# AKASH2907/pi-consistency-activity-detection

Measured on AMD Instinct MI355X. Metric: train clips/sec (bs=8, 16×224×224, I3D+caps+bv cons) at 1/2/4/8 GPU, higher is better.
Workload: dtype f32 (fp32 operands and fp32 accumulation everywhere; 33 of the 79 conv / input-gradient launches and the 3x3x3 / 1x1x1 weight gradients multiply on the bf16 matrix cores: every fp32 operand as the exact sum of 3 bf16 terms, 6 products on v_mfma_f32_32x32x16_bf16, hi / lo fp32 accumulators -- error v

## Files before the change

### include/picons.h

```cpp
#ifndef PICONS_H
#define PICONS_H
#include <stdint.h>
#ifdef __cplusplus
extern "C" {
#endif

typedef void* pc_stream;

#define PC_OK            0
#define PC_E_ARG        -1
#define PC_E_LAUNCH     -2
#define PC_E_NODEVICE   -3

#define PC_ACT_NONE 0
#define PC_ACT_RELU 1
#define PC_ACT_SIGMOID 2

#define PC_F_ACCUM   1
#define PC_F_BIAS    2
#define PC_F_CSCALE  4
#define PC_F_BNPART  8
#define PC_F_NFAST   16
#define PC_F_TOUT    32
#define PC_F_CI3     64
// ... 91 lines not shown
    pc_wgrad_desc d;
    const float* D; const float* S; float* g;
} pc_wgrad_job;
int pc_conv_wgrad_multi(const pc_wgrad_job* jobs, int njobs, pc_stream s);

int pc_bn_finalize(const float* part, int nparts_per_group, int groups, int C, int64_t count_per_group,
                   const float* gamma, const float* beta, float eps, float momentum,
                   float* running_mean, float* running_var, float* stat, pc_stream s);
int64_t pc_bn_finalize_ws_floats(int nparts_per_group, int groups, int C);
int pc_bn_finalize_ws(const float* part, int nparts_per_group, int groups, int C, int64_t count_per_group,
                      const float* gamma, const float* beta, float eps, float momentum,
                      float* running_mean, float* running_var, float* stat, float* ws, pc_stream s);
int pc_bn_apply(const float* z, int ldz, const float* stat, int C, int64_t rows, int groups, float* y,
                int ldy, int relu, pc_stream s);
int pc_bn_finalize_apply_ok(int nparts_per_group, int C);
int pc_bn_finalize_apply(const float* part, int nparts_per_group, int groups, int C, int64_t count_per_group, const float* gamma, const float* beta,
                         float eps, float momentum, float* running_mean, float* running_var, float* stat, const float* z, int ldz, int64_t rows,
                         float* y, int ldy, int relu, pc_stream s);
int pc_bn_eval_stat(const float* gamma, const float* beta, const float* running_mean,
                    const float* running_var, float eps, int C, float* stat, pc_stream s);
int64_t pc_bn_bwd_ws_floats(int64_t rows, int C, int groups);
int pc_bn_bwd(const float* dy, int lddy, const float* z, int ldz, const float* stat, int C,
              int64_t rows, int groups, int relu, float* dz, int lddz, float* dgamma, float* dbeta,
              int accum, float* ws, pc_stream s);

typedef struct pc_pool_desc {
    int32_t N, Ti, Hi, Wi, C, ldi;
    int32_t To, Ho, Wo, ldo;
    int32_t k[3], s[3], padf[3];
} pc_pool_desc;
int pc_maxpool_fwd(const pc_pool_desc* d, const float* x, float* y, uint8_t* argmax, pc_stream s);
int pc_maxpool_bwd(const pc_pool_desc* d, const float* dy, const uint8_t* argmax, float* dx,
                   int accum, pc_stream s);

int pc_channel_scale(const float* x, int ldx, const float* scale, int N, int64_t pos_per_n, int C,
                     float* y, int ldy, int accum, pc_stream s);
int64_t pc_act_bwd_ws_floats(int64_t rows, int C);
int pc_act_bwd(const float* dy, int lddy, const float* y, int ldy, int act, int C, int64_t rows,
               float* dz, int lddz, float* dbias, int accum, float* ws, pc_stream s);
int pc_ncdhw_to_ndhwc(const void* src, int src_is_f64, int N, int C, int64_t thw, int W, int Cpad,
                      int flipw, float* dst, pc_stream s);
int pc_ndhwc_to_ncdhw(const float* src, int ld, int N, int C, int64_t thw, float* dst, pc_stream s);
int pc_transpose_batched(const float* src, int batch, int R, int Cc, int64_t src_batch_stride,
                         int src_ld, float* dst, int64_t dst_batch_stride, int dst_ld, int accum,
                         pc_stream s);
typedef struct pc_transpose_job {
    uint64_t src, dst;
    int64_t  src_batch_stride, dst_batch_stride;
    int32_t  batch, R, C, src_ld, dst_ld, accum;
    int32_t  nslices, reserved;
    int64_t  slice_stride;
} pc_transpose_job;
int pc_transpose_multi(const pc_transpose_job* jobs, int njobs, pc_stream s);
int pc_col2im(const float* cols, int N, int Ho, int Wo, int KH, int KW, int C, float* dx, int lddx,
              int accum, pc_stream s);
int pc_seg_frame_counts(const float* logits, const float* gt, int64_t nframes, int64_t pix, int32_t* counts, pc_stream s);
int pc_map_accumulate(const int32_t* counts, int64_t nframes, int label, int ncls, int32_t* frame_hits, int32_t* video_hits,
                      int32_t* n_frames, int32_t* n_vids, pc_stream s);
int     pc_val_record_words(int B);
int64_t pc_val_metrics_ws_floats(int B, int64_t pix);
int     pc_val_metrics(const float* output, const float* loc_msk, const float* predicted_action, const int32_t* action, int B, int64_t pix,
                       int C, int32_t* record, float* ws, pc_stream s);
int pc_clip_from_u8(const uint8_t* video, int F, int H, int W, const int32_t* span8, int h0, int w0, int S,
                    const int32_t* rects, int R, float* data, float* aug, float* mask, pc_stream s);
int pc_clip_from_u8_masks(const uint8_t* video, int F, int H, int W, const int32_t* span8, int h0, int w0, int S,
                          const uint8_t* maskframes, const int32_t* valid8, float* data, float* aug, float* mask, float* mask_cls,
// ... 56 lines not shown
    float   bv_wt, gv_wt, wt_loc, wt_cons, wt_ramp;
} pc_loss_desc;
int64_t pc_loss_ws_floats(const pc_loss_desc* d);
int pc_consistency_loss(const pc_loss_desc* d, const float* output, const float* flip_op,
                        const float* seg, const int32_t* labeled, float* scalars, float* d_output,
                        float* d_flip_op, float* mask_bv, float* mask_gv, float* ws, pc_stream s);
int pc_var_mask(const float* pred, const float* flip_pred, int B, int T, int H, int W, int n_frames,
                int use_sig, float* mask, float* ws, pc_stream s);
int pc_grad_mask(const float* pred, int B, int T, int H, int W, float lower, float upper,
                 float* mask, float* ws, pc_stream s);
int pc_spread_loss(const float* x, const float* cls, const int32_t* labeled, int Bn, int C, float m,
                   float wt, float* out, float* dx, pc_stream s);

int pc_adam_step(float* p, const float* g, float* m, float* v, int64_t n, float lr, float b1,
                 float b2, float eps, int step, float gscale, pc_stream s);

typedef struct pc_axis_desc {
    int32_t R, I, O, C;
    int32_t in_split, out_split, act, act_c0, accum;
    int32_t in_sr, in_hi, in_lo, out_sr, out_hi, out_lo;
} pc_axis_desc;
int pc_axis_linear(const pc_axis_desc* d, const float* in, const float* M, const float* bias, float* out, pc_stream s);
int pc_wspec_fwd(const float* in, const float* tw, int A, int B, int KY, int KX, int U, int Ur, float* out, pc_stream s);
int pc_wspec_bwd(const float* dV, const float* tw, int A, int B, int KY, int KX, int U, int Ur, float* kg, pc_stream s);

int pc_wspec_master_fwd(const float* w, const float* tw, int Acnt, int a0, int Atot, int B, int KY, int KX, int U, int Ur,
                        float* out_f, float* out_t, pc_stream s);
int pc_wspec_master_planes(const float* w, const float* tw, int Acnt, int a0, int Atot, int B, int KY, int KX, int U, int Ur,
                           uint16_t* out_f, uint16_t* out_t, int64_t plane_stride, pc_stream s);
int pc_wspec_master_bwd(const float* dV, const float* tw, int Acnt, int a0, int Atot, int B, int KY, int KX, int U, int Ur,
                        float* dw, int accum, pc_stream s);

int pc_tail6_weights(const float* wf, int N, int Ci, float* W5f, float* W5t, pc_stream s);
int pc_tail6_gather(const float* cols, const float* bc, const float* bsm, int N, int It, int Ih, int Iw, float* out, pc_stream s);
int pc_tail6_scatter(const float* dout, int N, int It, int Ih, int Iw, float* dcols, pc_stream s);
int pc_tail6_wgrad_map(const float* dW5, int N, int Ci, float* Gc, pc_stream s);
int pc_tail6_wgrad_map_slices(float* ws, const int32_t* nslices8, int N, int Ci, float* Gc, pc_stream s);
int pc_tail6_bias_sums(const float* dout, int N, int It, int Ih, int Iw, float* sums, pc_stream s);
int64_t pc_tail6_bias_sums_ws_floats(int N, int It, int Ih, int Iw);
int pc_tail6_bias_sums_ws(const float* dout, int N, int It, int Ih, int Iw, float* sums, float* ws, pc_stream s);

typedef struct pc_op {
    int32_t  kind;
    int32_t  i[48];
    float    f[8];
    int32_t  lane;
    uint64_t p[12];
    int64_t  l[4];
} pc_op;
enum {
    PC_OP_CONV = 1, PC_OP_WGRAD, PC_OP_BN_FINALIZE, PC_OP_BN_APPLY, PC_OP_BN_EVAL_STAT, PC_OP_BN_BWD,
    PC_OP_POOL_FWD, PC_OP_POOL_BWD, PC_OP_CHSCALE, PC_OP_ACT_BWD, PC_OP_TO_NDHWC, PC_OP_TO_NCDHW,
    PC_OP_TRANSPOSE, PC_OP_FILL, PC_OP_AXPY, PC_OP_EM_FWD, PC_OP_EM_BWD, PC_OP_CMASK_FWD,
    PC_OP_CMASK_BWD, PC_OP_TAPSUM_FWD, PC_OP_TAPSUM_BWD, PC_OP_LOSS, PC_OP_SPREAD, PC_OP_ADAM,
    PC_OP_TAIL_COMBINE, PC_OP_TAIL_COLSUM, PC_OP_TAIL_GRADS, PC_OP_COL2IM,
    PC_OP_AXIS,
    PC_OP_WSPEC_FWD,
    PC_OP_WSPEC_BWD,
    PC_OP_WSPEC_MASTER_FWD,
    PC_OP_WSPEC_MASTER_BWD,
    PC_OP_TAIL6_WEIGHTS,
    PC_OP_TAIL6_GATHER,
    PC_OP_TAIL6_SCATTER,
    PC_OP_TAIL6_WGRAD_MAP,
    PC_OP_TAIL6_BIAS_SUMS,
    PC_OP_TRANSPOSE_MULTI,
// ... 28 lines not shown
```

### pi-consistency-activity-detection_amd/capi.py

```python
import ctypes as C
import os

import numpy as np

_HERE = os.path.dirname(os.path.abspath(__file__))
DIAG = os.environ.get("PICONS_DIAG_LIB", "0") not in ("", "0")
DIAG_SWITCHES = ("PICONS_CONV_ABLATE", "PICONS_WGRAD_ABLATE", "PICONS_WINO_VARIANT")
LIB_PATH = os.path.join(_HERE, "libpicons_diag.so" if DIAG else "libpicons.so")
if os.environ.get("PICONS_LIB_NAME"):
    LIB_PATH = os.path.join(_HERE, os.path.basename(os.environ["PICONS_LIB_NAME"]))
_lib = None

i32, i64, f32, vp = C.c_int32, C.c_int64, C.c_float, C.c_void_p


class ConvDesc(C.Structure):
    _fields_ = [(n, i32) for n in ("N", "Ti", "Hi", "Wi", "Ci", "ldi", "Tq", "Hq", "Wq", "To", "Ho", "Wo", "Co", "ldo")] + \
               [(n, i32 * 3) for n in ("ostr", "ooff", "istr", "ntap", "ioff0", "istep", "wk0", "wkstep")] + \
               [(n, i32) for n in ("KT", "KH", "KW", "ldw", "act", "flags", "wgstride", "bgstride", "act_c0", "groups")]


class WgradDesc(C.Structure):
    _fields_ = [(n, i32) for n in ("N", "Tq", "Hq", "Wq", "Cd", "ldd", "Ts", "Hs", "Ws", "Cs", "lds")] + \
               [(n, i32 * 3) for n in ("istr", "ntap", "ioff0", "istep", "wk0")] + [(n, i32) for n in ("KT", "KH", "KW", "splitk", "nbatch", "dbstride", "sbstride", "gbstride", "Td", "Hd", "Wd")] + [("doff", i32 * 3), ("flags", i32), ("ws_slices", i32)]
# ... 114 lines not shown
    "pc_clips_from_u8_views": (i32, [vp, i32, i32, i32, i32, C.POINTER(C.c_int32), i32, i32, C.POINTER(C.c_int32), i32, i32, vp, vp]),
    "pc_detect_frames_views_ws_bytes": (i64, [i32, i32, i32]),
    "pc_detect_frames_views": (i32, [vp, i32, i32, i32, i32, C.POINTER(C.c_int32), i32, i32, C.POINTER(C.c_int32), i32, i32, i32, vp, vp, vp, vp]),
    "pc_resize_tables": (i64, [i32, i32, i32, i32, i32, vp, i64]),
    "pc_resize_u8": (i32, [vp, i32, i32, i32, i32, i32, i32, vp, i32, vp, vp]),
    "pc_fill": (i32, [vp, i64, f32, vp]),
    "pc_axpy": (i32, [vp, vp, i64, f32, vp]),
    "pc_em_ws_floats": (i64, [i32, i32, i32]),
    "pc_em_state_floats": (i64, [i32]),
    "pc_em_routing_fwd": (i32, [vp, vp, vp, vp, i32, i32, i32, vp, vp, vp]),
    "pc_em_routing_bwd": (i32, [vp, vp, vp, vp, vp, i32, i32, i32, vp, vp, vp, vp, vp, vp, vp]),
    "pc_class_mask_fwd": (i32, [vp, i32, i32, i32, vp, vp, i32, vp, vp, vp, vp]),
    "pc_class_mask_bwd": (i32, [vp, vp, vp, i32, i32, i32, vp, vp]),
    "pc_tapsum_fwd": (i32, [vp, i32, i32, i32, i32, vp, vp, vp]),
    "pc_tapsum_bwd": (i32, [vp, i32, i32, i32, i32, vp, vp]),
    "pc_loss_ws_floats": (i64, [C.POINTER(LossDesc)]),
    "pc_consistency_loss": (i32, [C.POINTER(LossDesc), vp, vp, vp, vp, vp, vp, vp, vp, vp, vp, vp]),
    "pc_var_mask": (i32, [vp, vp, i32, i32, i32, i32, i32, i32, vp, vp, vp]),
    "pc_grad_mask": (i32, [vp, i32, i32, i32, i32, f32, f32, vp, vp, vp]),
    "pc_spread_loss": (i32, [vp, vp, vp, i32, i32, f32, f32, vp, vp, vp]),
    "pc_adam_step": (i32, [vp, vp, vp, vp, i64, f32, f32, f32, f32, i32, f32, vp]),
    "pc_tail_combine": (i32, [vp, vp, vp, vp, i32, i32, i32, i32, i32, vp, vp, vp, vp]),
    "pc_tail_colsum": (i32, [vp, i32, i64, vp, vp]),
    "pc_tail_grads": (i32, [vp, vp, vp, vp, vp, vp, i32, i32, i32, i32, i32, i32, vp, vp, vp, vp, i32, vp]),
    "pc_tail_grads_ws_floats": (i64, [i32, i32, i32]),
    "pc_tail_grads_ws": (i32, [vp, vp, vp, vp, vp, vp, i32, i32, i32, i32, i32, i32, vp, vp, vp, vp, i32, vp, vp]),
    "pc_axis_linear": (i32, [vp, vp, vp, vp, vp, vp]),
    "pc_wspec_fwd": (i32, [vp, vp, i32, i32, i32, i32, i32, i32, vp, vp]),
    "pc_wspec_bwd": (i32, [vp, vp, i32, i32, i32, i32, i32, i32, vp, vp]),
    "pc_wspec_master_fwd": (i32, [vp, vp, i32, i32, i32, i32, i32, i32, i32, i32, vp, vp, vp]),
    "pc_wspec_master_planes": (i32, [vp, vp, i32, i32, i32, i32, i32, i32, i32, i32, vp, vp, i64, vp]),
    "pc_wspec_master_bwd": (i32, [vp, vp, i32, i32, i32, i32, i32, i32, i32, i32, vp, i32, vp]),
    "pc_tail6_weights": (i32, [vp, i32, i32, vp, vp, vp]),
    "pc_tail6_gather": (i32, [vp, vp, vp, i32, i32, i32, i32, vp, vp]),
    "pc_tail6_scatter": (i32, [vp, i32, i32, i32, i32, vp, vp]),
    "pc_tail6_wgrad_map": (i32, [vp, i32, i32, vp, vp]),
    "pc_tail6_bias_sums": (i32, [vp, i32, i32, i32, i32, vp, vp]),
    "pc_tail6_wgrad_map_slices": (i32, [vp, vp, i32, i32, vp, vp]),
    "pc_tail6_bias_sums_ws_floats": (i64, [i32, i32, i32, i32]),
    "pc_tail6_bias_sums_ws": (i32, [vp, i32, i32, i32, i32, vp, vp, vp]),
    "pc_transpose_multi": (i32, [vp, i32, vp]),
    "pc_run_ops": (i32, [vp, i32, vp]),
    "pc_run_ops_lanes": (i32, [vp, i32, vp, i32]),
    "pc_streams_fanin": (i32, [vp, vp, i32]),
    "pc_release_thread_events": (i32, []),
    "pc_run_ops_timed": (i32, [vp, i32, i32, C.POINTER(f32), C.POINTER(i32), vp, i32]),
    "pc_run_ops_timed_collect": (i32, [C.POINTER(f32), C.POINTER(i32)]),
}
EXPORTS = sorted(_SIGS)


def lib():
    global _lib
    if _lib is None:
        stray = [k for k in DIAG_SWITCHES if os.environ.get(k, "0") not in ("", "0")]
        if stray and not DIAG:
            raise RuntimeError("%s set, but these switches exist only in the diagnostic build of the library (results can be wrong by design): "
                               "`make -C pi-consistency-activity-detection_amd/csrc diag` and PICONS_DIAG_LIB=1, or unset them" % ", ".join(stray))
        if not os.path.exists(LIB_PATH):
            raise RuntimeError("libpicons.so not built (%s): run `python -c 'import __graft_entry__ as g; g.build()'` "
                               "or `make -C pi-consistency-activity-detection_amd/csrc`; there is no CPU fallback" % LIB_PATH)
        L = C.CDLL(LIB_PATH)
        for name, (res, args) in _SIGS.items():
            fn = getattr(L, name)
            fn.restype = res
            fn.argtypes = args
# ... 27 lines not shown
```

### pi-consistency-activity-detection_amd/csrc/api.hip

```cpp
#include "common.h"
#include <string.h>
#include <vector>

static thread_local char g_err[512] = "";

void pc_set_error(const char* fmt, ...) {
    va_list ap;
    va_start(ap, fmt);
    vsnprintf(g_err, sizeof(g_err), fmt, ap);
    va_end(ap);
}

extern "C" const char* pc_last_error(void) { return g_err; }
extern "C" int pc_version(void) { return PC_VERSION; }

extern "C" int pc_transpose_batched(const float*, int, int, int, int64_t, int, float*, int64_t, int, int, pc_stream);

#define P(T, k) ((T)(uintptr_t)op.p[k])

static int run_one(const pc_op& op, pc_stream s) {
    switch (op.kind) {
        case PC_OP_CONV: {
            pc_conv_desc d;
            memcpy(&d, op.i, sizeof(d));
// ... 61 lines not shown
            return pc_transpose_batched(P(const float*, 0), op.i[0], op.i[1], op.i[2], op.l[0], op.i[3], P(float*, 1), op.l[1], op.i[4], op.i[5], s);
        case PC_OP_FILL:
            return pc_fill(P(float*, 0), op.l[0], op.f[0], s);
        case PC_OP_AXPY:
            return pc_axpy(P(float*, 0), P(const float*, 1), op.l[0], op.f[0], s);
        case PC_OP_EM_FWD:
            return pc_em_routing_fwd(P(const float*, 0), P(const float*, 1), P(const float*, 2), P(const float*, 3), op.i[0], op.i[1], op.i[2], P(float*, 4), P(float*, 5), s);
        case PC_OP_EM_BWD:
            return pc_em_routing_bwd(P(const float*, 0), P(const float*, 1), P(const float*, 2), P(const float*, 3), P(const float*, 4), op.i[0], op.i[1],
                                     op.i[2], P(float*, 5), P(float*, 6), P(float*, 7), P(float*, 8), P(float*, 9), P(const float*, 10), s);
        case PC_OP_CMASK_FWD:
            return pc_class_mask_fwd(P(const float*, 0), op.i[0], op.i[1], op.i[2], P(const float*, 1), P(const int32_t*, 2), op.i[3], P(float*, 3),
                                     P(float*, 4), P(float*, 5), s);
        case PC_OP_CMASK_BWD:
            return pc_class_mask_bwd(P(const float*, 0), P(const float*, 1), P(const float*, 2), op.i[0], op.i[1], op.i[2], P(float*, 3), s);
        case PC_OP_TAPSUM_FWD:
            return pc_tapsum_fwd(P(const float*, 0), op.i[0], op.i[1], op.i[2], op.i[3], P(const float*, 1), P(float*, 2), s);
        case PC_OP_TAPSUM_BWD:
            return pc_tapsum_bwd(P(const float*, 0), op.i[0], op.i[1], op.i[2], op.i[3], P(float*, 1), s);
        case PC_OP_LOSS: {
            pc_loss_desc d;
            d.B = op.i[0]; d.T = op.i[1]; d.H = op.i[2]; d.W = op.i[3]; d.bv = op.i[4]; d.gv = op.i[5]; d.n_frames = op.i[6];
            d.predict_maps = op.i[7]; d.jhmdb = op.i[8];
            d.lower_thresh = op.f[0]; d.upper_thresh = op.f[1]; d.bv_wt = op.f[2]; d.gv_wt = op.f[3]; d.wt_loc = op.f[4];
            d.wt_cons = op.f[5]; d.wt_ramp = op.f[6];
            return pc_consistency_loss(&d, P(const float*, 0), P(const float*, 1), P(const float*, 2), P(const int32_t*, 3), P(float*, 4), P(float*, 5),
                                       P(float*, 6), P(float*, 7), P(float*, 8), P(float*, 9), s);
        }
        case PC_OP_SPREAD:
            return pc_spread_loss(P(const float*, 0), P(const float*, 1), P(const int32_t*, 2), op.i[0], op.i[1], op.f[0], op.f[1], P(float*, 3), P(float*, 4), s);
        case PC_OP_ADAM:
            return pc_adam_step(P(float*, 0), P(const float*, 1), P(float*, 2), P(float*, 3), op.l[0], op.f[0], op.f[1], op.f[2], op.f[3], op.i[0], op.f[4], s);
        case PC_OP_TAIL_COMBINE:
            return pc_tail_combine(P(const float*, 0), P(const float*, 1), P(const float*, 2), P(const float*, 3), op.i[0], op.i[1], op.i[2], op.i[3],
                                   op.i[4], P(float*, 4), P(float*, 5), P(float*, 6), s);
        case PC_OP_TAIL_COLSUM:
            return pc_tail_colsum(P(const float*, 0), op.i[0], op.l[0], P(float*, 1), s);
        case PC_OP_TAIL_GRADS:
            return pc_tail_grads_ws(P(const float*, 0), P(const float*, 1), P(const float*, 2), P(const float*, 3), P(const float*, 4), P(const float*, 5),
                                    op.i[0], op.i[1], op.i[2], op.i[3], op.i[4], op.i[5], P(float*, 6), P(float*, 7), P(float*, 8), P(float*, 9), op.i[6],
                                    P(float*, 10), s);
        case PC_OP_COL2IM:
            return pc_col2im(P(const float*, 0), op.i[0], op.i[1], op.i[2], op.i[3], op.i[4], op.i[5], P(float*, 1), op.i[6], op.i[7], s);
        case PC_OP_AXIS: {
            pc_axis_desc d;
            memcpy(&d, op.i, sizeof(d));
            return pc_axis_linear(&d, P(const float*, 0), P(const float*, 1), P(const float*, 2), P(float*, 3), s);
        }
        case PC_OP_WSPEC_FWD:
            return pc_wspec_fwd(P(const float*, 0), P(const float*, 1), op.i[0], op.i[1], op.i[2], op.i[3], op.i[4], op.i[5], P(float*, 2), s);
        case PC_OP_WSPEC_BWD:
            return pc_wspec_bwd(P(const float*, 0), P(const float*, 1), op.i[0], op.i[1], op.i[2], op.i[3], op.i[4], op.i[5], P(float*, 2), s);
        case PC_OP_WSPEC_MASTER_FWD:
            return pc_wspec_master_fwd(P(const float*, 0), P(const float*, 1), op.i[0], op.i[1], op.i[2], op.i[3], op.i[4], op.i[5], op.i[6], op.i[7],
                                       P(float*, 2), P(float*, 3), s);
        case PC_OP_WSPEC_MASTER_BWD:
            return pc_wspec_master_bwd(P(const float*, 0), P(const float*, 1), op.i[0], op.i[1], op.i[2], op.i[3], op.i[4], op.i[5], op.i[6], op.i[7],
                                       P(float*, 2), op.i[8], s);
        case PC_OP_TAIL6_WEIGHTS:
            return pc_tail6_weights(P(const float*, 0), op.i[0], op.i[1], P(float*, 1), P(float*, 2), s);
        case PC_OP_TAIL6_GATHER:
            return pc_tail6_gather(P(const float*, 0), P(const float*, 1), P(const float*, 2), op.i[0], op.i[1], op.i[2], op.i[3], P(float*, 3), s);
        case PC_OP_TAIL6_SCATTER:
            return pc_tail6_scatter(P(const float*, 0), op.i[0], op.i[1], op.i[2], op.i[3], P(float*, 1), s);
        case PC_OP_TAIL6_WGRAD_MAP:
            return op.i[2] ? pc_tail6_wgrad_map_slices(P(float*, 0), &op.i[3], op.i[0], op.i[1], P(float*, 1), s)
// ... 178 lines not shown
```

### pi-consistency-activity-detection_amd/csrc/tail6.hip

```cpp
#include "common.h"
#include <stdlib.h>

namespace {

constexpr int NSLOT = 125, SP = 128, J32 = 32;

__device__ __forceinline__ int npairs(int k5, bool first) { return k5 == 0 || k5 == 4 ? 1 : (k5 == 2 ? (first ? 2 : 3) : 2); }
__device__ __forceinline__ int pair_k4(int k5, bool first, int q) {
    switch (k5) {
        case 0: return 0;
        case 1: return q;
        case 2: return first ? 1 + q : q;
        case 3: return 1 + q;
        default: return 2;
    }
}

__global__ __launch_bounds__(256) void tail6_weights_kernel(const float* __restrict__ wf, int N, int Ci, float* __restrict__ W5f,
                                                            float* __restrict__ W5t) {
    const int64_t total = (int64_t)N * 8 * SP * Ci;
    for (int64_t idx = (int64_t)blockIdx.x * 256 + threadIdx.x; idx < total; idx += (int64_t)gridDim.x * 256) {
        const int ci = (int)(idx % Ci);
        const int slot = (int)((idx / Ci) % SP);
        const int z = (int)((idx / ((int64_t)Ci * SP)) % 8);
        const int n = (int)(idx / ((int64_t)Ci * SP * 8));
        float acc = 0.f;
        if (slot < NSLOT) {
            const int st = slot / 25, sh = (slot / 5) % 5, sw = slot % 5;
            const bool ft = z & 4, fh = z & 2, fw = z & 1;
            const float* base = wf + (size_t)n * J32 * 27 * Ci + ci;
            for (int a = 0; a < npairs(st, ft); ++a)
                for (int b = 0; b < npairs(sh, fh); ++b)
                    for (int c = 0; c < npairs(sw, fw); ++c) {
                        const int ka = pair_k4(st, ft, a), kb = pair_k4(sh, fh, b), kc = pair_k4(sw, fw, c);
                        const int tap = (ka * 3 + kb) * 3 + kc;
                        const int j = ((st - ka) * 3 + (sh - kb)) * 3 + (sw - kc);
                        acc += base[((size_t)j * 27 + tap) * Ci];
                    }
        }
        W5f[idx] = acc;
        W5t[(((size_t)n * 8 + z) * Ci + ci) * SP + slot] = acc;
    }
}

__device__ __forceinline__ int dim_terms(int o, int I, int (&ii)[3], int (&kk)[3]) {
    int n = 0;
#pragma unroll
    for (int k5 = 0; k5 < 5; ++k5) {
        const int t = o + 2 - k5;
        if (t >= 0 && !(t & 1) && (t >> 1) < I) { ii[n] = t >> 1; kk[n] = k5; ++n; }
    }
    return n;
}

__global__ __launch_bounds__(256) void tail6_gather_kernel(const float* __restrict__ cols, const float* __restrict__ bc, const float* __restrict__ bsm,
                                                           int N, int It, int Ih, int Iw, float* __restrict__ out) {
    const int Ot = 2 * It, Oh = 2 * Ih, Ow = 2 * Iw;
    const int64_t total = (int64_t)N * Ot * Oh * Ow;
    const int64_t idx = (int64_t)blockIdx.x * 256 + threadIdx.x;
    if (idx >= total) return;
    const int ow = (int)(idx % Ow), oh = (int)((idx / Ow) % Oh), ot = (int)((idx / ((int64_t)Ow * Oh)) % Ot), n = (int)(idx / ((int64_t)Ow * Oh * Ot));
    int it[3], kt[3], ih[3], kh[3], iw[3], kw[3];
    const int nt = dim_terms(ot, It, it, kt), nh = dim_terms(oh, Ih, ih, kh), nw = dim_terms(ow, Iw, iw, kw);
    float acc = bsm[0];
    for (int a = 0; a < 3; ++a) {
        const int mt = ot + 1 - a;
        if (mt < 0 || mt >= Ot) continue;
        for (int b = 0; b < 3; ++b) {
            const int mh = oh + 1 - b;
            if (mh < 0 || mh >= Oh) continue;
            for (int c = 0; c < 3; ++c) {
                const int mw = ow + 1 - c;
                if (mw < 0 || mw >= Ow) continue;
                acc += bc[n * J32 + (a * 3 + b) * 3 + c];
            }
        }
    }
// ... 171 lines not shown
        else atomicAdd(sums + n * J32 + threadIdx.x, v);
    }
}

__global__ __launch_bounds__(32) void tail6_bias_sums_final_kernel(const float* __restrict__ part, int nb, float* __restrict__ sums) {
    const int n = blockIdx.x, j = threadIdx.x;
    float v = 0.f;
    if (j < 27) {
        const float* q = part + (size_t)n * nb * J32 + j;
        int b = 0;
        for (; b + 14 <= nb; b += 14) {
            float t[14];
#pragma unroll
            for (int u = 0; u < 14; ++u) t[u] = q[(size_t)(b + u) * J32];
#pragma unroll
            for (int u = 0; u < 14; ++u) v += t[u];
        }
        for (; b < nb; ++b) v += q[(size_t)b * J32];
    }
    sums[n * J32 + j] = v;
}

}

extern "C" int pc_tail6_weights(const float* wf, int N, int Ci, float* W5f, float* W5t, pc_stream s) {
    PC_CHECK_ARG(wf && W5f && W5t && N >= 1 && Ci >= 1, "pc_tail6_weights: bad args");
    const int64_t total = (int64_t)N * 8 * SP * Ci;
    int grid = (int)((total + 255) / 256); if (grid > 8192) grid = 8192;
    hipLaunchKernelGGL(tail6_weights_kernel, dim3(grid), dim3(256), 0, (hipStream_t)s, wf, N, Ci, W5f, W5t);
    PC_CHECK_LAUNCH("tail6_weights");
    return PC_OK;
}

extern "C" int pc_tail6_gather(const float* cols, const float* bc, const float* bsm, int N, int It, int Ih, int Iw, float* out, pc_stream s) {
    PC_CHECK_ARG(cols && bc && bsm && out && N >= 1 && It >= 1 && Ih >= 1 && Iw >= 1, "pc_tail6_gather: bad args");
    const int64_t total = (int64_t)N * 8 * It * Ih * Iw;
    PC_CHECK_ARG((total + 255) / 256 < (1ll << 31), "pc_tail6_gather: too large");
    if (((uintptr_t)out & 7) == 0) {
        const dim3 grid((unsigned)((int64_t)N * It * Ih));
        hipLaunchKernelGGL((tail6_gather_rows_kernel<0, 0>), grid, dim3(128), 0, (hipStream_t)s, cols, bc, bsm, N, It, Ih, Iw, out);
        hipLaunchKernelGGL((tail6_gather_rows_kernel<0, 1>), grid, dim3(128), 0, (hipStream_t)s, cols, bc, bsm, N, It, Ih, Iw, out);
        hipLaunchKernelGGL((tail6_gather_rows_kernel<1, 0>), grid, dim3(128), 0, (hipStream_t)s, cols, bc, bsm, N, It, Ih, Iw, out);
        hipLaunchKernelGGL((tail6_gather_rows_kernel<1, 1>), grid, dim3(128), 0, (hipStream_t)s, cols, bc, bsm, N, It, Ih, Iw, out);
    } else {
        hipLaunchKernelGGL(tail6_gather_kernel, dim3((unsigned)cdiv(total, 256)), dim3(256), 0, (hipStream_t)s, cols, bc, bsm, N, It, Ih, Iw, out);
    }
    PC_CHECK_LAUNCH("tail6_gather");
    return PC_OK;
}

extern "C" int pc_tail6_scatter(const float* dout, int N, int It, int Ih, int Iw, float* dcols, pc_stream s) {
    PC_CHECK_ARG(dout && dcols && N >= 1 && It >= 1 && Ih >= 1 && Iw >= 1, "pc_tail6_scatter: bad args");
    const int64_t total = (int64_t)N * It * Ih * Iw * (SP / 4);
    PC_CHECK_ARG((total + 255) / 256 < (1ll << 31), "pc_tail6_scatter: too large");
    hipLaunchKernelGGL(tail6_scatter_kernel, dim3((unsigned)cdiv(total, 256)), dim3(256), 0, (hipStream_t)s, dout, N, It, Ih, Iw, dcols);
    PC_CHECK_LAUNCH("tail6_scatter");
    return PC_OK;
}

static int t6_wgrad_map(float* dW5, const int32_t* nslices8, int N, int Ci, float* Gc, pc_stream s) {
    PC_CHECK_ARG(dW5 && Gc && N >= 1 && Ci >= 1, "pc_tail6_wgrad_map: bad args");
    T6Slices sl;
    sl.image = nslices8 ? (long long)N * Ci * SP : 0;
    long long at = 0;
    for (int z = 0; z < 8; ++z) {
        sl.n[z] = nslices8 ? nslices8[z] : 1;
// ... 55 lines not shown
```

### pi-consistency-activity-detection_amd/ops.py

```python
import ctypes as C

import numpy as np
import torch

from . import capi, desc as D


def stream():
    return C.c_void_p(torch.cuda.current_stream().cuda_stream)


def ptr(t):
    if t is None:
        return None
    if not t.is_cuda:
        raise RuntimeError("picons ops need CUDA/HIP tensors (no CPU fallback)")
    return C.c_void_p(t.data_ptr())


def _fill_struct(st, d):
    for name, ctype in st._fields_:
        v = d[name]
        if isinstance(v, (list, tuple)):
            setattr(st, name, (C.c_int32 * 3)(*[int(x) for x in v]))
# ... 278 lines not shown
def spread_loss(x, cls, labeled, m=0.2, wt=1.0, dx=None):
    out = torch.empty(2, device=x.device)
    capi.call("pc_spread_loss", ptr(x), ptr(cls), ptr(labeled), x.shape[0], x.shape[1], m, wt, ptr(out), ptr(dx), stream())
    return out


def adam_step(p, g, m, v, lr, step, b1=0.9, b2=0.999, eps=1e-6, gscale=1.0):
    capi.call("pc_adam_step", ptr(p), ptr(g), ptr(m), ptr(v), p.numel(), lr, b1, b2, eps, step, gscale, stream())


def axis_linear(d, x, M, out, bias=None):
    st = capi.AxisDesc(*[int(d[k]) for k in capi.AXIS_FIELDS])
    capi.call("pc_axis_linear", C.byref(st), ptr(x), ptr(M), ptr(bias), ptr(out), stream())
    return out


def wspec_fwd(w, tw, A, B, KY, KX, U, Ur, out):
    capi.call("pc_wspec_fwd", ptr(w), ptr(tw), A, B, KY, KX, U, Ur, ptr(out), stream())
    return out


def wspec_bwd(dV, tw, A, B, KY, KX, U, Ur, kg):
    capi.call("pc_wspec_bwd", ptr(dV), ptr(tw), A, B, KY, KX, U, Ur, ptr(kg), stream())
    return kg


def wspec_master_fwd(w, tw, Acnt, a0, Atot, B, KY, KX, U, Ur, out_f, out_t):
    capi.call("pc_wspec_master_fwd", ptr(w), ptr(tw), Acnt, a0, Atot, B, KY, KX, U, Ur, ptr(out_f), ptr(out_t), stream())


def wspec_master_bwd(dV, tw, Acnt, a0, Atot, B, KY, KX, U, Ur, dw, accum=False):
    capi.call("pc_wspec_master_bwd", ptr(dV), ptr(tw), Acnt, a0, Atot, B, KY, KX, U, Ur, ptr(dw), int(accum), stream())
    return dw


def tail6_weights(wf, N, Ci, W6f, W6t):
    capi.call("pc_tail6_weights", ptr(wf), N, Ci, ptr(W6f), ptr(W6t), stream())


def tail6_gather(cols, bc, bsm, N, It, Ih, Iw, out):
    capi.call("pc_tail6_gather", ptr(cols), ptr(bc), ptr(bsm), N, It, Ih, Iw, ptr(out), stream())
    return out


def tail6_scatter(dout, N, It, Ih, Iw, dcols):
    capi.call("pc_tail6_scatter", ptr(dout), N, It, Ih, Iw, ptr(dcols), stream())
    return dcols


def tail6_wgrad_map(dW6, N, Ci, Gc):
    capi.call("pc_tail6_wgrad_map", ptr(dW6), N, Ci, ptr(Gc), stream())
    return Gc


def tail6_bias_sums(dout, N, It, Ih, Iw, sums, ws=None):
    if ws is None:
        capi.call("pc_tail6_bias_sums", ptr(dout), N, It, Ih, Iw, ptr(sums), stream())
    else:
        assert ws.numel() >= tail6_bias_sums_ws_floats(N, It, Ih, Iw)
        capi.call("pc_tail6_bias_sums_ws", ptr(dout), N, It, Ih, Iw, ptr(sums), ptr(ws), stream())
    return sums


def tail6_bias_sums_ws_floats(N, It, Ih, Iw):
    return int(capi.lib().pc_tail6_bias_sums_ws_floats(N, It, Ih, Iw))

# ... 324 lines not shown
```

### pi-consistency-activity-detection_amd/plan.py

```python
from dataclasses import dataclass, field

import os

import numpy as np

from . import capi, desc as D, spec, spectral, switches as sw, tail6

ALIGN = 256


@dataclass
class TR:
    ref: tuple
    N: int
    thw: tuple
    C: int
    ld: int
    name: str = ""

    @property
    def rows(self):
        return self.N * self.thw[0] * self.thw[1] * self.thw[2]

    def slice(self, c0, c):
# ... 9 lines not shown

class Plan:
    def __init__(self, num_classes=24, hw=224, n=4, groups=2, training=True, jhmdb=False, accum_grads=False, lanes=1, spectral_pc=None,
                 early_adam=False, exp=None):
        self.acc = 1 if accum_grads else 0
        self.exp = dict(exp or {})
        self.early_adam = bool(early_adam) and lanes >= 2 and training and sw.get("PICONS_EARLY_ADAM", "1") != "0"
        self.op_adam_early, self.adam_split = None, 0
        if hw % 8 or hw // 8 < spec.PRIMARY_K:
            raise ValueError("frame size %d: must be a multiple of 8 and at least %d (the 9x9 PrimaryCaps conv needs a feature map of "
                             "9x9 or more)" % (hw, 8 * spec.PRIMARY_K))
        if not 1 <= lanes <= capi.MAX_LANES:
            raise ValueError("lanes must be 1..%d" % capi.MAX_LANES)
        self.lanes = lanes
        self.lane = 0
        want_skip = sw.get("PICONS_SKIP_LANE", "1") != "0" and lanes >= 3
        want_wg = sw.get("PICONS_WGRAD_LANE", "1") != "0" and lanes >= 3
        own_wg = want_wg and want_skip and lanes >= 4 and sw.get("PICONS_WGRAD_SEPARATE", "1") != "0"
        self.wg_lane = lanes - 1 if want_wg else 0
        self.skip_lane = (lanes - 2 if own_wg else lanes - 1) if want_skip else 0
        self.branch_lanes = lanes - len({ln for ln in (self.wg_lane, self.skip_lane) if ln})
        self.skip_bwd = {}
        self.final_lane = {}
        self.deferred = None
        self.after_bn_bwd = None
        self.wgrad_collect = None
        self.wg_ordered = sw.get("PICONS_WGRAD_ATOMIC", "0") == "0"
        self.spectral_pc = (sw.get("PICONS_SPECTRAL", "1") != "0") if spectral_pc is None else bool(spectral_pc)
        self.x6 = sw.get("PICONS_SPLIT", "1") != "0"
        self.wbufs = []
        self.consts = []
        self.zero_once = []
        self.merged_tail = sw.get("PICONS_TAIL6", "1") != "0"
        self.spread_classes = lanes >= 2 and sw.get("PICONS_SPREAD_CLASSES", "1") != "0"
        self.conv28_aside = sw.get("PICONS_CONV28_ASIDE", "1") != "0"
        self.C = num_classes
        self.hw = hw
        self.n = n
        self.groups = groups
        self.N = n * groups
        self.training = training
        self.jhmdb = jhmdb
        self.arena_bytes = 0
        self.lists = {"prep": [], "prep_late": [], "fwd": [], "loss": [], "bwd": [], "unprep": [], "adam": []}
        self.late_prep = bool(self.wg_lane) and sw.get("PICONS_LATE_PREP", "1") != "0"
        self.prep_target = "prep_late" if self.late_prep else "prep"
        self.cur = "fwd"
        self.tape = []
        self.grads = {}
        self.kw = {}
        self.named = {}
        self.pshape = spec.param_shapes(num_classes)
        self.fuse_1x1 = sw.get("PICONS_FUSE1X1", "1") != "0"
        self.fused_groups = ([["conv1.%s.%s" % (ent[0], b) for b in ("b1a", "b2a", "b0")] for ent in spec.TRUNK if ent[1] == "mixed"]
                             if self.fuse_1x1 else [])
        head = {g[2] + ".conv3d.weight": g for g in self.fused_groups}
        grouped = {pre + sfx for g in self.fused_groups for pre in g for sfx in (".conv3d.weight", ".bn.weight", ".bn.bias")}
        order = []
        for k in self.pshape:
            if k in head:
                order += [pre + sfx for sfx in (".conv3d.weight", ".bn.weight", ".bn.bias") for pre in head[k]]
            elif k not in grouped:
                order.append(k)
        assert sorted(order) == sorted(self.pshape)
        self.poff = {}
        o = 0
# ... 758 lines not shown
        for g in range(self.groups):
            self.op_to_ndhwc.append(len(self.lists["fwd"]))
            src = self.in_data if g == 0 else self.in_aug
            self.emit(capi.OP_TO_NDHWC, i=[0, self.n, 3, hw, 4, 0], l=[T * hw * hw], p=[src, off(x.ref, g * self.n * T * hw * hw * 4)])
        out56 = out112 = None
        first = True
        s28e = hw // 8
        if self.skip_lane:
            cat56 = self.tensor(N, (2, 2 * s28e, 2 * s28e), 128, "cat56")
            cat112 = self.tensor(N, (4, 4 * s28e, 4 * s28e), 128, "cat112")
        pending_skip, skip_after = [], sw.exp("PICONS_SKIP_FWD_AFTER", "", self.exp)
        for ent in spec.TRUNK:
            name = "conv1." + ent[0]
            if ent[0] == "Mixed_3b" and self.late_prep:
                self.join(1 << self.wg_lane)
            if ent[1] == "conv":
                x = self.unit3d(name, x, ent[3], ent[4], ent[5], need_dx=not first)
                first = False
            elif ent[1] == "pool":
                x = self.maxpool(x, ent[2], ent[3], name)
            else:
                x = self.inception(name, x, ent[3])
            if ent[0] == "Conv3d_2c_3x3":
                out56 = x
                if self.skip_lane:
                    pending_skip.append(("conv56", out56, cat56))
            if ent[0] == "Conv3d_1a_7x7":
                out112 = x
                if self.skip_lane:
                    pending_skip.append(("conv112", out112, cat112))
            if pending_skip and (not skip_after or ent[0] == skip_after or ent is spec.TRUNK[-1]):
                for nm_, t_, c_ in pending_skip:
                    self._skip_conv(nm_, t_, c_)
                pending_skip = []
            if ent[0] == "MaxPool3d_3a_3x3" and self.skip_lane:
                inner = self.tape.pop()
                self.tape.append(lambda inner=inner: (self.join(1 << self.skip_lane), inner()))
        self.named["trunk_out"] = x
        s28 = x.thw[1]
        if self.training:
            xd = self.tensor(N, x.thw, x.C, "x832d")
            self.emit(capi.OP_CHSCALE, i=[x.ld, N, x.C, xd.ld, 0], l=[x.rows // N], p=[x.ref, self.in_drop832, xd.ref])
            xin = x

            def bwd_drop():
                dxd = self.grad_of(xd)
                dx, acc = self.grad_for_write(xin)
                self.emit(capi.OP_CHSCALE, i=[dxd.ld, N, xin.C, dx.ld, int(acc)], l=[xin.rows // N], p=[dxd.ref, self.in_drop832, dx.ref])
            self.tape.append(bwd_drop)
        else:
            xd = x
        cat28 = self.tensor(N, (1, s28, s28), 128, "cat28")
        conv28_early = bool(self.conv28_aside and self.skip_lane)
        if conv28_early:
            self.fork(1 << self.skip_lane)
            self.lane = self.skip_lane
            self.conv_layer("conv28", xd, 64, (1, 3, 3), (0, 1, 1), capi.ACT_RELU, cat28.slice(64, 64))
            self.lane = 0
            self.skip_bwd["conv28"] = self.tape.pop()
        KP = spec.PRIMARY_K
        s20 = s28 - KP + 1
        npose = spec.IN_CAPS * spec.POSE
        caps_in = self.tensor(N, (1, s20, s20), npose + spec.IN_CAPS, "caps_in")
        spectral_pc = self.spectral_pc and xd.thw[0] == 1
        pc_dgrad_wv = False
        Cpc = npose + spec.IN_CAPS
# ... 99 lines not shown
                dg = D.conv_fwd(N, caps_in.thw, caps_in.C, dcaps.ld, KP * KP * xd.C, KP * KP * xd.C, (1, 1, 1), (1, 1, 1), (0, 0, 0),
                                caps_in.thw, ldw=caps_in.C)
                self.conv_op(dg, dcaps.ref, wpc["tio"], cols, alg=F_pc)
                self.emit(capi.OP_COL2IM, i=[N, caps_in.thw[1], caps_in.thw[2], KP, KP, xd.C, dx.ld, int(acc)], p=[cols, dx.ref])
            else:
                self.alg_dgrad(F_pc)
                for dd in D.transposed_classes(N, caps_in.thw, caps_in.C, dcaps.ld, xd.thw, xd.C, dx.ld, (1, KP, KP), (1, 1, 1), (0, 0, 0),
                                               flags=(capi.F_ACCUM if acc else 0) | capi.F_NFAST, ldw=caps_in.C):
                    self.conv_op(dd, dcaps.ref, wpc["tr"], dx.ref, alg=0)
        self.tape.append(bwd_caps)
        self.convT_layer("upsample1", masked, 64, (1, KP, KP), (1, 1, 1), (0, 0, 0), (0, 0, 0), capi.ACT_RELU, cat28.slice(0, 64))
        if conv28_early:
            self.tape.append(self.skip_bwd["conv28"])
            self.join(1 << self.skip_lane)
        else:
            self.conv_layer("conv28", xd, 64, (1, 3, 3), (0, 1, 1), capi.ACT_RELU, cat28.slice(64, 64))
        if not self.skip_lane:
            cat56 = self.tensor(N, (2, 2 * s28, 2 * s28), 128, "cat56")
        self.convT_layer("upsample2", cat28, 64, (3, 3, 3), (2, 2, 2), (1, 1, 1), (1, 1, 1), capi.ACT_RELU, cat56.slice(0, 64))
        if self.skip_lane:
            self.tape.append(self._on_skip_lane(self.skip_bwd["conv56"]))
            self.join(1 << self.skip_lane)
        else:
            self.conv_layer("conv56", out56, 64, (3, 3, 3), (1, 1, 1), capi.ACT_RELU, cat56.slice(64, 64))
            cat112 = self.tensor(N, (4, 4 * s28, 4 * s28), 128, "cat112")
        self.convT_layer("upsample3", cat56, 64, (3, 3, 3), (2, 2, 2), (1, 1, 1), (1, 1, 1), capi.ACT_RELU, cat112.slice(0, 64))
        if self.skip_lane:
            self.tape.append(self._on_skip_lane(self.skip_bwd["conv112"]))
        else:
            self.conv_layer("conv112", out112, 64, (3, 3, 3), (1, 1, 1), capi.ACT_RELU, cat112.slice(64, 64))
        othw = (8, 8 * s28, 8 * s28)
        k3, s2, p1 = (3, 3, 3), (2, 2, 2), (1, 1, 1)
        J = 27
        wt = self.alloc(N * 128 * 27 * 32)
        wf = self.alloc(N * 32 * 27 * 128)
        bc = self.alloc(N * 32)
        cs_ref = self.in_drop128 if self.training else None
        W4, b4, Wp = self.P("upsample4.weight"), self.P("upsample4.bias"), self.P("smooth.weight")
        self.emit(capi.OP_TAIL_COMBINE, i=[N, 128, 128, 27, J], p=[W4, b4, cs_ref, Wp, wt, wf, bc])
        if self.merged_tail:
            return self._merged_tail(cat112, othw, wf, bc, cs_ref, W4, b4, Wp, J)
        proj = self.tensor(N, othw, 32, "proj")
        F_tail = 0
        for dd in D.transposed_classes(N, cat112.thw, 128, cat112.ld, othw, 32, 32, k3, s2, p1, flags=capi.F_BIAS, groups=N):
            dd["wgstride"] = 32 * 27 * 128
            dd["bgstride"] = 32
            dd["Co_real"] = J
            F_tail += _conv_flops(dd)
            self.conv_op(dd, cat112.ref, wf, proj.ref, bias=bc)
        out = self.tensor(N, othw, 1, "out")
        self.emit(capi.OP_TAPSUM_FWD, i=[N, othw[0], othw[1], othw[2]], p=[proj.ref, self.P("smooth.bias"), out.ref])
        self.out = out

        def bwd_smooth():
            dproj = self.tensor(N, othw, 32, "d_proj")
            self.emit(capi.OP_TAPSUM_BWD, i=[N, othw[0], othw[1], othw[2]], p=[self.dout, dproj.ref])
            sums = self.alloc(N * 32)
            per_n = othw[0] * othw[1] * othw[2]
            self.emit(capi.OP_TAIL_COLSUM, i=[N], l=[per_n], p=[dproj.ref, sums])
            Gc = self.alloc(N * 128 * 27 * 32)
            self.emit(capi.OP_FILL, p=[Gc], l=[N * 128 * 27 * 32], f=[0.0])
            xin_per = cat112.thw[0] * cat112.thw[1] * cat112.thw[2] * cat112.ld
            wd = D.trim_wgrad(D.wgrad(1, cat112.thw, 128, cat112.ld, othw, 32, 32, k3, s2, p1))
            wd.update(nbatch=N, dbstride=xin_per, sbstride=per_n * 32, gbstride=128 * 27 * 32, Cs_real=J)
            self.wgrad_op(wd, [cat112.ref, dproj.ref, Gc])
            self.emit(capi.OP_TAIL_GRADS, i=[N, 128, 128, 27, J, 13, self.acc],
                      p=[Gc, sums, W4, b4, cs_ref, Wp, self.G("upsample4.weight"), self.G("upsample4.bias"), self.G("smooth.weight"), self.G("smooth.bias")])
            self.mark_final("upsample4.weight", "upsample4.bias", "smooth.weight", "smooth.bias")
            dx, acc = self.grad_for_write(cat112)
            dd = D.conv_fwd(N, othw, 32, 32, 128, dx.ld, k3, s2, p1, cat112.thw, flags=capi.F_ACCUM if acc else 0, groups=N, ldw=32)
            dd["wgstride"] = 128 * 27 * 32
            dd["Ci_real"] = J
            self.conv_op(dd, dproj.ref, wt, dx.ref, alg=F_tail)
        self.tape.append(bwd_smooth)
        return out

    def _merged_tail(self, cat112, othw, wf, bc, cs_ref, W4, b4, Wp, J):
        N = cat112.N
        It, Ih, Iw = cat112.thw
        SP = tail6.SP
        w5f = self.alloc(N * 8 * SP * 128)
        w5t = self.alloc(N * 8 * 128 * SP)
        self.emit(capi.OP_TAIL6_WEIGHTS, i=[N, 128], p=[wf, w5f, w5t])
        self.reg_weight(w5f, N * 8 * SP * 128)
        self.reg_weight(w5t, N * 8 * 128 * SP)
        if self.x6:
            self.planes_of(w5f)
            self.planes_of(w5t)
        cols = self.alloc(cat112.rows * SP)
        F_t6 = 2 * cat112.rows * 125 * 128
        self.fork()
        for q, (z, d) in enumerate(tail6.conv_descs(N, cat112.thw, 128, cat112.ld)):
            self.lane = 0 if z == 0 else 1 % self.branch_lanes
            self.conv_op(d, cat112.ref, off(w5f, z * SP * 128), cols, alg=F_t6 if q == 0 else 0)
        self.lane = 0
        self.join()
        out = self.tensor(N, othw, 1, "out")
        self.emit(capi.OP_TAIL6_GATHER, i=[N, It, Ih, Iw], p=[cols, bc, self.P("smooth.bias"), out.ref])
        self.out = out

        def bwd_smooth():
            dcols = self.alloc(cat112.rows * SP)
            self.emit(capi.OP_TAIL6_SCATTER, i=[N, It, Ih, Iw], p=[self.dout, dcols])
            sums = self.alloc(N * 32)
            sums_ws = self.alloc(capi.lib().pc_tail6_bias_sums_ws_floats(N, It, Ih, Iw)) if self.wg_ordered else 0
            self.emit(capi.OP_TAIL6_BIAS_SUMS, i=[N, It, Ih, Iw], p=[self.dout, sums, sums_ws])
            wds = tail6.wgrad_descs(N, cat112.thw, 128, cat112.ld, compact=self.wg_ordered)
            ns8, zoff = [0] * 8, {}
            if self.wg_ordered:
                at = 0
                for z, wd in wds:
                    if self.x6 and sw.get("PICONS_SPLIT_WGRAD", "1") != "0":
                        wd["flags"] = int(wd.get("flags", 0)) | capi.WG_X6
                    ns8[z] = capi.lib().pc_wgrad_slices(_wdesc(wd))
                    if ns8[z] < 1:
                        raise RuntimeError("pc_wgrad_slices: %s" % capi.lib().pc_last_error().decode())
                    wd["ws_slices"] = ns8[z]
                    zoff[z] = at
                    at += ns8[z] * N * 128 * SP
                dW5 = self.alloc(at)
                self.zero_once.append((dW5, at))
# ... 351 lines not shown
```

Before: 433.4.

## Fuse tail weight combine, tail6 weight build and bf16 plane split into one kernel

Adds a single kernel that combines the upsample4 and smooth weights, builds the merged-tail W5f/W5t weights and writes their 3-term bf16 planes in one pass, instead of separate combine, tail6-weights and plane-split launches. The planner emits this kernel early on the skip lane right after conv56, so it can overlap with trunk work. This removes launches and intermediate round-trips through global memory for small weight tensors. In exchange the kernel is specialised to 27 taps and at most 128 middle channels, and the plane buffers are now allocated by hand.

```diff
diff --git a/include/picons.h b/include/picons.h
--- a/include/picons.h
+++ b/include/picons.h
@@ -147,6 +147,7 @@
 int pc_maxpool_fwd(const pc_pool_desc* d, const float* x, float* y, uint8_t* argmax, pc_stream s);
 int pc_maxpool_bwd(const pc_pool_desc* d, const float* dy, const uint8_t* argmax, float* dx,
                    int accum, pc_stream s);
+
 
 int pc_channel_scale(const float* x, int ldx, const float* scale, int N, int64_t pos_per_n, int C,
                      float* y, int ldy, int accum, pc_stream s);
@@ -269,6 +270,8 @@
                         float* dw, int accum, pc_stream s);
 
 int pc_tail6_weights(const float* wf, int N, int Ci, float* W5f, float* W5t, pc_stream s);
+int pc_tail_weights(const float* W4, const float* b4, const float* cs, const float* Wp, int N, int Ci, int Co, int taps, int J, float* Wt, float* Wf,
+                    float* bc, float* W5f, float* W5t, uint16_t* P5f, uint16_t* P5t, int64_t plane_stride, pc_stream s);
 int pc_tail6_gather(const float* cols, const float* bc, const float* bsm, int N, int It, int Ih, int Iw, float* out, pc_stream s);
 int pc_tail6_scatter(const float* dout, int N, int It, int Ih, int Iw, float* dcols, pc_stream s);
 int pc_tail6_wgrad_map(const float* dW5, int N, int Ci, float* Gc, pc_stream s);
diff --git a/pi-consistency-activity-detection_amd/capi.py b/pi-consistency-activity-detection_amd/capi.py
--- a/pi-consistency-activity-detection_amd/capi.py
+++ b/pi-consistency-activity-detection_amd/capi.py
@@ -170,6 +170,7 @@
     "pc_wspec_master_planes": (i32, [vp, vp, i32, i32, i32, i32, i32, i32, i32, i32, vp, vp, i64, vp]),
     "pc_wspec_master_bwd": (i32, [vp, vp, i32, i32, i32, i32, i32, i32, i32, i32, vp, i32, vp]),
     "pc_tail6_weights": (i32, [vp, i32, i32, vp, vp, vp]),
+    "pc_tail_weights": (i32, [vp, vp, vp, vp, i32, i32, i32, i32, i32, vp, vp, vp, vp, vp, vp, vp, i64, vp]),
     "pc_tail6_gather": (i32, [vp, vp, vp, i32, i32, i32, i32, vp, vp]),
     "pc_tail6_scatter": (i32, [vp, i32, i32, i32, i32, vp, vp]),
     "pc_tail6_wgrad_map": (i32, [vp, i32, i32, vp, vp]),
diff --git a/pi-consistency-activity-detection_amd/csrc/api.hip b/pi-consistency-activity-detection_amd/csrc/api.hip
--- a/pi-consistency-activity-detection_amd/csrc/api.hip
+++ b/pi-consistency-activity-detection_amd/csrc/api.hip
@@ -117,6 +117,9 @@
         case PC_OP_ADAM:
             return pc_adam_step(P(float*, 0), P(const float*, 1), P(float*, 2), P(float*, 3), op.l[0], op.f[0], op.f[1], op.f[2], op.f[3], op.i[0], op.f[4], s);
         case PC_OP_TAIL_COMBINE:
+            if (op.i[5])
+                return pc_tail_weights(P(const float*, 0), P(const float*, 1), P(const float*, 2), P(const float*, 3), op.i[0], op.i[1], op.i[2], op.i[3], op.i[4],
+                                       P(float*, 4), P(float*, 5), P(float*, 6), P(float*, 7), P(float*, 8), P(uint16_t*, 9), P(uint16_t*, 10), op.l[0], s);
             return pc_tail_combine(P(const float*, 0), P(const float*, 1), P(const float*, 2), P(const float*, 3), op.i[0], op.i[1], op.i[2], op.i[3],
                                    op.i[4], P(float*, 4), P(float*, 5), P(float*, 6), s);
         case PC_OP_TAIL_COLSUM:
diff --git a/pi-consistency-activity-detection_amd/csrc/tail6.hip b/pi-consistency-activity-detection_amd/csrc/tail6.hip
--- a/pi-consistency-activity-detection_amd/csrc/tail6.hip
+++ b/pi-consistency-activity-detection_amd/csrc/tail6.hip
@@ -1,4 +1,4 @@
-#include "common.h"
+#include "conv_common.h"
 #include <stdlib.h>
 
 namespace {
@@ -43,6 +43,97 @@
     }
 }
 
+constexpr int TW_CB = 4, TW_CO = 128, TW_T = 27;
+__global__ __launch_bounds__(256) void tail_weights_kernel(const float* __restrict__ W4, const float* __restrict__ b4, const float* __restrict__ cs,
+                                                           const float* __restrict__ Wp, int Ci, int Co, float* __restrict__ Wt, float* __restrict__ Wf,
+                                                           float* __restrict__ bc, float* __restrict__ W5f, float* __restrict__ W5t,
+                                                           uint16_t* __restrict__ P5f, uint16_t* __restrict__ P5t, long long pstride) {
+    __shared__ __attribute__((aligned(16))) float sWp[TW_CO * TW_T];
+    __shared__ __attribute__((aligned(16))) float sW4[TW_CO * TW_T];
+    __shared__ float sSc[TW_CO];
+    __shared__ float sWc[TW_CB][TW_T][TW_T];
+    __shared__ __attribute__((aligned(16))) float sW5[8][TW_CB][SP];
+    const int tid = threadIdx.x, n = blockIdx.y, ci0 = blockIdx.x * TW_CB;
+    for (int e = tid; e < Co * TW_T; e += 256) sWp[e] = Wp[e];
+    for (int e = tid; e < Co; e += 256) sSc[e] = cs ? cs[n * Co + e] : 1.f;
+    __syncthreads();
+    if (blockIdx.x == 0 && tid < J32) {
+        float acc = 0.f;
+        if (tid < TW_T)
+            for (int co = 0; co < Co; ++co) acc += b4[co] * sSc[co] * sWp[co * TW_T + tid];
+        bc[n * J32 + tid] = acc;
+    }
+    for (int cl = 0; cl < TW_CB; ++cl) {
+        const float* w4 = W4 + (size_t)(ci0 + cl) * Co * TW_T;
+        for (int e = tid; e < Co * TW_T; e += 256) sW4[e] = w4[e] * sSc[e / TW_T];
+        __syncthreads();
+        for (int o = tid; o < TW_T * TW_T; o += 256) {
+            const int tap = o / TW_T, j = o - tap * TW_T;
+            float acc = 0.f;
+            for (int co = 0; co < Co; ++co) acc += sW4[co * TW_T + tap] * sWp[co * TW_T + j];
+            sWc[cl][tap][j] = acc;
+        }
+        __syncthreads();
+    }
+    if (Wt) {
+        float* o = Wt + ((size_t)n * Ci + ci0) * TW_T * J32;
+        for (int e = tid; e < TW_CB * TW_T * J32; e += 256) {
+            const int j = e & 31, tap = (e >> 5) % TW_T, cl = e / (TW_T * J32);
+            o[e] = j < TW_T ? sWc[cl][tap][j] : 0.f;
+        }
+    }
+    for (int e = tid; e < J32 * TW_T; e += 256) {
+        const int j = e / TW_T, tap = e - j * TW_T;
+        f32x4 v = {0.f, 0.f, 0.f, 0.f};
+        if (j < TW_T) v = f32x4{sWc[0][tap][j], sWc[1][tap][j], sWc[2][tap][j], sWc[3][tap][j]};
+        *(f32x4*)(Wf + (((size_t)n * J32 + j) * TW_T + tap) * Ci + ci0) = v;
+    }
+    for (int e = tid; e < 8 * SP; e += 256) {
+        const int z = e / SP, slot = e - z * SP;
+        f32x4 v = {0.f, 0.f, 0.f, 0.f};
+        if (slot < NSLOT) {
+            const int st = slot / 25, sh = (slot / 5) % 5, sw = slot % 5;
+            const bool ft = z & 4, fh = z & 2, fw = z & 1;
+            for (int a = 0; a < npairs(st, ft); ++a)
+                for (int b = 0; b < npairs(sh, fh); ++b)
+                    for (int c = 0; c < npairs(sw, fw); ++c) {
+                        const int ka = pair_k4(st, ft, a), kb = pair_k4(sh, fh, b), kc = pair_k4(sw, fw, c);
+                        const int tap = (ka * 3 + kb) * 3 + kc;
+                        const int j = ((st - ka) * 3 + (sh - kb)) * 3 + (sw - kc);
+#pragma unroll
+                        for (int cl = 0; cl < TW_CB; ++cl) v[cl] += sWc[cl][tap][j];
+                    }
+        }
+#pragma unroll
+        for (int cl = 0; cl < TW_CB; ++cl) sW5[z][cl][slot] = v[cl];
+        const size_t at = (((size_t)n * 8 + z) * SP + slot) * Ci + ci0;
+        *(f32x4*)(W5f + at) = v;
+        if (P5f) {
+            uint32_t h0, m0, l0, h1, m1, l1;
+            x6_split2(v[0], v[1], h0, m0, l0);
+            x6_split2(v[2], v[3], h1, m1, l1);
+            *(uint2*)(P5f + at) = make_uint2(h0, h1);
+            *(uint2*)(P5f + pstride + at) = make_uint2(m0, m1);
+            *(uint2*)(P5f + 2 * pstride + at) = make_uint2(l0, l1);
+        }
+    }
+    __syncthreads();
+    for (int e = tid; e < 8 * TW_CB * (SP / 4); e += 256) {
+        const int s4 = e % (SP / 4), cl = (e / (SP / 4)) % TW_CB, z = e / (TW_CB * (SP / 4));
+        const f32x4 v = *(const f32x4*)&sW5[z][cl][s4 * 4];
+        const size_t at = (((size_t)n * 8 + z) * Ci + ci0 + cl) * SP + s4 * 4;
+        *(f32x4*)(W5t + at) = v;
+        if (P5t) {
+            uint32_t h0, m0, l0, h1, m1, l1;
+            x6_split2(v[0], v[1], h0, m0, l0);
+            x6_split2(v[2], v[3], h1, m1, l1);
+            *(uint2*)(P5t + at) = make_uint2(h0, h1);
+            *(uint2*)(P5t + pstride + at) = make_uint2(m0, m1);
+            *(uint2*)(P5t + 2 * pstride + at) = make_uint2(l0, l1);
+        }
+    }
+}
+
 __device__ __forceinline__ int dim_terms(int o, int I, int (&ii)[3], int (&kk)[3]) {
     int n = 0;
 #pragma unroll
@@ -280,6 +371,20 @@
     return PC_OK;
 }
 
+extern "C" int pc_tail_weights(const float* W4, const float* b4, const float* cs, const float* Wp, int N, int Ci, int Co, int taps, int J, float* Wt, float* Wf,
+                               float* bc, float* W5f, float* W5t, uint16_t* P5f, uint16_t* P5t, int64_t plane_stride, pc_stream s) {
+    PC_CHECK_ARG(W4 && b4 && Wp && Wf && bc && W5f && W5t && N >= 1 && N <= 65535, "pc_tail_weights: bad args");
+    PC_CHECK_ARG(taps == TW_T && J == TW_T && Co >= 1 && Co <= TW_CO && Ci >= TW_CB && Ci % TW_CB == 0,
+                 "pc_tail_weights: built for 27 taps, 27 smooth taps, at most %d middle channels and a multiple of %d input channels (taps=%d J=%d Co=%d Ci=%d)",
+                 TW_CO, TW_CB, taps, J, Co, Ci);
+    PC_CHECK_ARG((P5f == nullptr) == (P5t == nullptr) && (!P5f || (plane_stride >= (int64_t)N * 8 * SP * Ci && plane_stride % 4 == 0)),
+                 "pc_tail_weights: the planes of W5f and W5t go together, %lld elements apart at least", (long long)((int64_t)N * 8 * SP * Ci));
+    PC_CHECK_ARG(((uintptr_t)Wf | (uintptr_t)W5f | (uintptr_t)W5t) % 16 == 0 && ((uintptr_t)P5f | (uintptr_t)P5t) % 8 == 0, "pc_tail_weights: outputs must be 16-byte (planes 8-byte) aligned");
+    hipLaunchKernelGGL(tail_weights_kernel, dim3(Ci / TW_CB, N), dim3(256), 0, (hipStream_t)s, W4, b4, cs, Wp, Ci, Co, Wt, Wf, bc, W5f, W5t, P5f, P5t, (long long)plane_stride);
+    PC_CHECK_LAUNCH("tail_weights");
+    return PC_OK;
+}
+
 extern "C" int pc_tail6_gather(const float* cols, const float* bc, const float* bsm, int N, int It, int Ih, int Iw, float* out, pc_stream s) {
     PC_CHECK_ARG(cols && bc && bsm && out && N >= 1 && It >= 1 && Ih >= 1 && Iw >= 1, "pc_tail6_gather: bad args");
     const int64_t total = (int64_t)N * 8 * It * Ih * Iw;
diff --git a/pi-consistency-activity-detection_amd/ops.py b/pi-consistency-activity-detection_amd/ops.py
--- a/pi-consistency-activity-detection_amd/ops.py
+++ b/pi-consistency-activity-detection_amd/ops.py
@@ -334,6 +334,11 @@
 def wspec_master_bwd(dV, tw, Acnt, a0, Atot, B, KY, KX, U, Ur, dw, accum=False):
     capi.call("pc_wspec_master_bwd", ptr(dV), ptr(tw), Acnt, a0, Atot, B, KY, KX, U, Ur, ptr(dw), int(accum), stream())
     return dw
+
+
+def tail_weights(W4, b4, cs, Wp, N, Ci, Co, Wt, Wf, bc, W5f, W5t, P5f=None, P5t=None, plane_stride=0):
+    capi.call("pc_tail_weights", ptr(W4), ptr(b4), ptr(cs), ptr(Wp), N, Ci, Co, 27, 27, ptr(Wt), ptr(Wf), ptr(bc), ptr(W5f), ptr(W5t), ptr(P5f), ptr(P5t),
+              int(plane_stride), stream())
 
 
 def tail6_weights(wf, N, Ci, W6f, W6t):
diff --git a/pi-consistency-activity-detection_amd/plan.py b/pi-consistency-activity-detection_amd/plan.py
--- a/pi-consistency-activity-detection_amd/plan.py
+++ b/pi-consistency-activity-detection_amd/plan.py
@@ -65,6 +65,8 @@
         self.consts = []
         self.zero_once = []
         self.merged_tail = sw.get("PICONS_TAIL6", "1") != "0"
+        self.tail_fused = self.merged_tail and sw.get("PICONS_TAIL_WEIGHTS_FUSED", "1") != "0"
+        self.tailw = None
         self.spread_classes = lanes >= 2 and sw.get("PICONS_SPREAD_CLASSES", "1") != "0"
         self.conv28_aside = sw.get("PICONS_CONV28_ASIDE", "1") != "0"
         self.C = num_classes
@@ -889,6 +891,10 @@
             if pending_skip and (not skip_after or ent[0] == skip_after or ent is spec.TRUNK[-1]):
                 for nm_, t_, c_ in pending_skip:
                     self._skip_conv(nm_, t_, c_)
+                    if nm_ == "conv56" and self.tail_fused:
+                        self.lane = self.skip_lane
+                        self._tail_weights_fused()
+                        self.lane = 0
                 pending_skip = []
             if ent[0] == "MaxPool3d_3a_3x3" and self.skip_lane:
                 inner = self.tape.pop()
@@ -1054,11 +1060,15 @@
         othw = (8, 8 * s28, 8 * s28)
         k3, s2, p1 = (3, 3, 3), (2, 2, 2), (1, 1, 1)
         J = 27
+        cs_ref = self.in_drop128 if self.training else None
+        W4, b4, Wp = self.P("upsample4.weight"), self.P("upsample4.bias"), self.P("smooth.weight")
+        if self.tail_fused:
+            if self.tailw is None:
+                self._tail_weights_fused()
+            return self._merged_tail(cat112, othw, self.tailw["wf"], self.tailw["bc"], cs_ref, W4, b4, Wp, J)
         wt = self.alloc(N * 128 * 27 * 32)
         wf = self.alloc(N * 32 * 27 * 128)
         bc = self.alloc(N * 32)
-        cs_ref = self.in_drop128 if self.training else None
-        W4, b4, Wp = self.P("upsample4.weight"), self.P("upsample4.bias"), self.P("smooth.weight")
         self.emit(capi.OP_TAIL_COMBINE, i=[N, 128, 128, 27, J], p=[W4, b4, cs_ref, Wp, wt, wf, bc])
         if self.merged_tail:
             return self._merged_tail(cat112, othw, wf, bc, cs_ref, W4, b4, Wp, J)
@@ -1097,18 +1107,39 @@
         self.tape.append(bwd_smooth)
         return out
 
+    def _tail_weights_fused(self):
+        N, SP = self.N, tail6.SP
+        wf = self.alloc(N * 32 * 27 * 128)
+        bc = self.alloc(N * 32)
+        w5f = self.alloc(N * 8 * SP * 128)
+        w5t = self.alloc(N * 8 * 128 * SP)
+        nw = N * 8 * SP * 128
+        planes = []
+        for ref in (w5f, w5t):
+            self.reg_weight(ref, nw)
+            if self.x6:
+                self._wbuf_of(ref)["planes"] = self.alloc((3 * nw + 1) // 2)
+            planes.append(self._wbuf_of(ref)["planes"])
+        cs_ref = self.in_drop128 if self.training else None
+        self.emit(capi.OP_TAIL_COMBINE, i=[N, 128, 128, 27, 27, 1], l=[nw],
+                  p=[self.P("upsample4.weight"), self.P("upsample4.bias"), cs_ref, self.P("smooth.weight"), None, wf, bc, w5f, w5t] + planes)
+        self.tailw = dict(wf=wf, bc=bc, w5f=w5f, w5t=w5t)
+
     def _merged_tail(self, cat112, othw, wf, bc, cs_ref, W4, b4, Wp, J):
         N = cat112.N
         It, Ih, Iw = cat112.thw
         SP = tail6.SP
-        w5f = self.alloc(N * 8 * SP * 128)
-        w5t = self.alloc(N * 8 * 128 * SP)
-        self.emit(capi.OP_TAIL6_WEIGHTS, i=[N, 128], p=[wf, w5f, w5t])
-        self.reg_weight(w5f, N * 8 * SP * 128)
-        self.reg_weight(w5t, N * 8 * 128 * SP)
-        if self.x6:
-            self.planes_of(w5f)
-            self.planes_of(w5t)
+        if self.tailw is not None:
+            w5f, w5t = self.tailw["w5f"], self.tailw["w5t"]
+        else:
+            w5f = self.alloc(N * 8 * SP * 128)
+            w5t = self.alloc(N * 8 * 128 * SP)
+            self.emit(capi.OP_TAIL6_WEIGHTS, i=[N, 128], p=[wf, w5f, w5t])
+            self.reg_weight(w5f, N * 8 * SP * 128)
+            self.reg_weight(w5t, N * 8 * 128 * SP)
+            if self.x6:
+                self.planes_of(w5f)
+                self.planes_of(w5t)
         cols = self.alloc(cat112.rows * SP)
         F_t6 = 2 * cat112.rows * 125 * 128
         self.fork()
```

After: 437.5 (median of 6 runs). About the same (+0.9%).
